# leotimus/binary-recommendation

Measured on NVIDIA B200. Metric: train interactions/sec (BPR, d=64, ML-1M shape), higher is better.
Workload: dtype f32

## Files before the change

binary-recommendation_b200/csrc/bpr.cu:

```cuda
#include "neumf_common.cuh"
#include <cooperative_groups.h>
#include <stdlib.h>
#include <vector>

namespace {

constexpr int kThreads = 256;

__device__ __forceinline__ uint32_t peek_touched(const uint32_t* touched, int64_t row) {
  return touched ? __ldg(touched + (row >> 5)) : 0xffffffffu;
}
__device__ __forceinline__ void mark_touched(uint32_t* touched, int64_t row, uint32_t seen) {
  const uint32_t bit = 1u << (row & 31);
  if (!(seen & bit)) atomicOr(touched + (row >> 5), bit);
}

__device__ __forceinline__ void finish_loss(double part, double inv_batch, double* acc, unsigned int* ticket,
                                            float* loss_out) {
  __shared__ double red[32];
  const double tot = block_sum_double(part, red);
  if (threadIdx.x == 0) {
    atomicAdd(acc, tot);
    __threadfence();
    const unsigned int t = atomicAdd(ticket, 1u);
    if (t == gridDim.x - 1) {
      __threadfence();
      const double sum = atomicAdd(acc, 0.0);
      if (loss_out) loss_out[0] = float(sum * inv_batch);
      *acc = 0.0;
      *ticket = 0u;
      __threadfence();
    }
  }
// ... 169 lines not shown
}

struct BprStep {
  int64_t off;
  int64_t sample_index;
  int32_t count;
  int32_t _pad;
};
constexpr int kInlineSteps = 16;
struct BprCoopParams {
  brk_table user, item;
  const int32_t* u; const int32_t* p; const int32_t* n;
  const BprStep* steps;
  BprStep inline_steps[kInlineSteps];
  int32_t use_inline;
  int32_t n_steps;
  brk_adam_hyper h;
  int64_t* state;
  float* losses;
  double* loss_acc;
  int32_t* stage;
  int64_t stage_pitch;
  const int64_t* csr_indptr; const int32_t* csr_items;
  uint32_t seed, epoch, num_items;
  float* const* peer_w; float* const* peer_g; uint32_t* const* peer_flags;
  float* dp_m; float* dp_v; uint32_t* dp_sync;
  int64_t arena_n4;
  int32_t rank, world;
  float inv_global;
  unsigned long long* dbg;
  long long spin_budget;
  int32_t prefetch;
  unsigned int* bar;
};

__device__ __forceinline__ void coop_st_release_sys(uint32_t* p, uint32_t v) {
  asm volatile("st.release.sys.global.u32 [%0], %1;" ::"l"(p), "r"(v) : "memory");
}
__device__ __forceinline__ bool coop_spin_sys(const uint32_t* p, uint32_t epoch, uint32_t* err, long long budget) {
  const long long t0 = clock64();
  while (true) {
    uint32_t v;
    asm volatile("ld.acquire.sys.global.u32 %0, [%1];" : "=r"(v) : "l"(p) : "memory");
    if (int32_t(v - epoch) >= 0) return true;
    if (clock64() - t0 > budget) { atomicExch(err, 1u); return false; }
    __nanosleep(32);
  }
}

__device__ __forceinline__ void coop_stamp(const BprCoopParams& P, int s, int k) {
  if (P.dbg && blockIdx.x == 0 && threadIdx.x == 0) {
    unsigned long long t;
    asm volatile("mov.u64 %0, %globaltimer;" : "=l"(t));
    P.dbg[s * 8 + k] = t;
  }
}

__device__ __forceinline__ void adam4(float4& w, float4& m, float4& v, const float4 g, float alpha, float b1, float b2,
                                      float eps) {
  const float omb1 = 1.f - b1, omb2 = 1.f - b2;
  m.x = b1 * m.x + omb1 * g.x; v.x = b2 * v.x + omb2 * g.x * g.x; w.x -= alpha * m.x / (sqrtf(v.x) + eps);
  m.y = b1 * m.y + omb1 * g.y; v.y = b2 * v.y + omb2 * g.y * g.y; w.y -= alpha * m.y / (sqrtf(v.y) + eps);
  m.z = b1 * m.z + omb1 * g.z; v.z = b2 * v.z + omb2 * g.z * g.z; w.z -= alpha * m.z / (sqrtf(v.z) + eps);
  m.w = b1 * m.w + omb1 * g.w; v.w = b2 * v.w + omb2 * g.w * g.w; w.w -= alpha * m.w / (sqrtf(v.w) + eps);
}

__device__ __forceinline__ void bpr_stage_step(const BprCoopParams& P, const BprStep sd, int slot, int64_t tid, int64_t nthr) {
  int32_t* su = P.stage + int64_t(slot) * 3 * P.stage_pitch;
  int32_t* sp = su + P.stage_pitch; int32_t* sn = sp + P.stage_pitch;
  for (int64_t b = tid; b < sd.count; b += nthr) {
    const int32_t uu = P.u[sd.off + b];
    su[b] = uu; sp[b] = P.p[sd.off + b];
    sn[b] = brk_sample_bpr_negative(uint64_t(sd.sample_index + b), uu, P.seed, P.epoch, P.num_items, P.csr_indptr, P.csr_items);
  }
}

constexpr int kStageThreads = 64;

template <int LPR, int NCH>
__global__ void __launch_bounds__(kThreads, 4) bpr_steps_coop(const BprCoopParams P) {
  namespace cg = cooperative_groups;
  cg::grid_group grid = cg::this_grid();
  unsigned int bar_target = P.bar ? *reinterpret_cast<volatile unsigned int*>(P.bar + 2) : 0u;
  auto gsync = [&]() {
    if (P.bar == nullptr) { grid.sync(); return; }
    __syncthreads();
    bar_target += gridDim.x;
    if (threadIdx.x == 0) {
      asm volatile("red.release.gpu.global.add.u32 [%0], 1;" ::"l"(P.bar) : "memory");
      const long long t0 = clock64();
      unsigned int v;
      do {
        asm volatile("ld.acquire.gpu.global.u32 %0, [%1];" : "=r"(v) : "l"(P.bar) : "memory");
        if (clock64() - t0 > 8000000000LL) { atomicExch(P.bar + 1, 1u); __trap(); }
      } while (int(v - bar_target) < 0);
    }
    __syncthreads();
  };
  auto gcollect = [&]() {
    if (P.bar == nullptr) { grid.sync(); return; }
    __syncthreads();
    bar_target += gridDim.x;
    if (threadIdx.x == 0) {
      asm volatile("red.release.gpu.global.add.u32 [%0], 1;" ::"l"(P.bar) : "memory");
      if (blockIdx.x == 0) {
        const long long t0 = clock64();
        unsigned int v;
        do {
          asm volatile("ld.acquire.gpu.global.u32 %0, [%1];" : "=r"(v) : "l"(P.bar) : "memory");
          if (clock64() - t0 > 8000000000LL) { atomicExch(P.bar + 1, 1u); __trap(); }
        } while (int(v - bar_target) < 0);
      }
    }
    if (blockIdx.x == 0) __syncthreads();
  };
  __shared__ double red[32];
  const bool sample = P.n == nullptr;
  const int d4 = P.user.d >> 2;
  const int lane_in = threadIdx.x & (LPR - 1);
  const int sub = (threadIdx.x & 31) / LPR;
  const int64_t group = (int64_t(blockIdx.x) * kThreads + threadIdx.x) / LPR;
  const int64_t n_groups = int64_t(gridDim.x) * kThreads / LPR;
  const int64_t warp_first = group - sub;
  const int64_t tid = int64_t(blockIdx.x) * kThreads + threadIdx.x, nthr = int64_t(gridDim.x) * kThreads;
  const float4* Wu4 = reinterpret_cast<const float4*>(P.user.w);
  const float4* Wi4 = reinterpret_cast<const float4*>(P.item.w);
  const double* pw = reinterpret_cast<const double*>(P.state);
  double p1 = pw[1], p2 = pw[2];
  const brk_table tabs[2] = {P.user, P.item};

  if (P.prefetch && threadIdx.x == 0) {
    for (int k = 0; k < 2; ++k) {
      const int64_t bytes = tabs[k].rows * tabs[k].d * 4;
      int64_t per = (bytes + gridDim.x - 1) / gridDim.x;
      per = (per + 15) & ~int64_t(15);
      const int64_t off = int64_t(blockIdx.x) * per;
      if (off < bytes) {
        const uint32_t n = uint32_t(((off + per <= bytes ? per : bytes - off)) & ~int64_t(15));
        if (n) {
          const float* arrs[4] = {tabs[k].w, tabs[k].g, P.world > 1 ? nullptr : tabs[k].m, P.world > 1 ? nullptr : tabs[k].v};
#pragma unroll
          for (int a = 0; a < 4; ++a)
            if (arrs[a] != nullptr && brk_aligned16(arrs[a]))
              asm volatile("cp.async.bulk.prefetch.L2.global [%0], %1;" ::"l"(reinterpret_cast<const char*>(arrs[a]) + off), "r"(n) : "memory");
        }
      }
    }
  }
  if (sample) {
    bpr_stage_step(P, P.use_inline ? P.inline_steps[0] : P.steps[0], 0, tid, nthr);
    gsync();
  }
  for (int s = 0; s < P.n_steps; ++s) {
    const BprStep sd = P.use_inline ? P.inline_steps[s] : P.steps[s];
    const int64_t batch = sd.count;
    const float inv_batch = P.world > 1 ? P.inv_global : 1.0f / float(batch);
    coop_stamp(P, s, 0);
    const int32_t *uid, *pid, *nid;
    if (sample) { uid = P.stage + int64_t(s & 1) * 3 * P.stage_pitch; pid = uid + P.stage_pitch; nid = pid + P.stage_pitch; }
    else { uid = P.u + sd.off; pid = P.p + sd.off; nid = P.n + sd.off; }
    float loss_local = 0.f;
    for (int64_t wb = warp_first; wb < batch; wb += n_groups) {
      const int64_t b = wb + sub;
      const bool valid = b < batch;
      int64_t ru = 0, rp = 0, rn = 0;
      if (valid) { ru = __ldcg(uid + b); rp = __ldcg(pid + b); rn = __ldcg(nid + b); }
      float4 u[NCH], p[NCH], n[NCH];
#pragma unroll
      for (int k = 0; k < NCH; ++k) {
        const int c = lane_in + k * LPR;
        if (valid && c < d4) {
          u[k] = __ldcg(Wu4 + ru * d4 + c); p[k] = __ldcg(Wi4 + rp * d4 + c); n[k] = __ldcg(Wi4 + rn * d4 + c);
        } else {
          u[k] = p[k] = n[k] = make_float4(0.f, 0.f, 0.f, 0.f);
        }
      }
      float dot = 0.f;
#pragma unroll
      for (int k = 0; k < NCH; ++k) {
        dot = fmaf(u[k].x, p[k].x - n[k].x, dot); dot = fmaf(u[k].y, p[k].y - n[k].y, dot);
        dot = fmaf(u[k].z, p[k].z - n[k].z, dot); dot = fmaf(u[k].w, p[k].w - n[k].w, dot);
      }
      const float x = group_sum<LPR>(dot);
      const float sg = sigmoidf_acc(x);
      if (valid && lane_in == 0) loss_local += 1.0f - sg;
      const float g = -sg * (1.0f - sg) * inv_batch;
      if (valid) {
#pragma unroll
        for (int k = 0; k < NCH; ++k) {
          const int c = lane_in + k * LPR;
          if (c < d4) {
            const float4 dp = make_float4(g * u[k].x, g * u[k].y, g * u[k].z, g * u[k].w);
            red_add_f4(P.user.g + (ru * d4 + c) * 4, make_float4(g * (p[k].x - n[k].x), g * (p[k].y - n[k].y),
                                                                 g * (p[k].z - n[k].z), g * (p[k].w - n[k].w)));
            red_add_f4(P.item.g + (rp * d4 + c) * 4, dp);
            red_add_f4(P.item.g + (rn * d4 + c) * 4, make_float4(-dp.x, -dp.y, -dp.z, -dp.w));
          }
        }
      }
    }
    const double part = block_sum_double(double(loss_local), red);
    if (threadIdx.x == 0) atomicAdd(P.loss_acc + (s & 1), part);
    if (P.world > 1) gcollect(); else gsync();
    coop_stamp(P, s, 1);
    p1 *= double(P.h.beta1); p2 *= double(P.h.beta2);
    const float alpha = float(double(P.h.lr) * sqrt(1.0 - p2) / (1.0 - p1));
    const bool staging = sample && s + 1 < P.n_steps;
    const bool stager = staging && threadIdx.x < kStageThreads;
    const int64_t atid = staging ? int64_t(blockIdx.x) * (kThreads - kStageThreads) + (threadIdx.x - kStageThreads) : tid;
    const int64_t anthr = staging ? int64_t(gridDim.x) * (kThreads - kStageThreads) : nthr;
    if (stager) {
      bpr_stage_step(P, P.use_inline ? P.inline_steps[s + 1] : P.steps[s + 1], (s + 1) & 1,
                     int64_t(blockIdx.x) * kStageThreads + threadIdx.x, int64_t(gridDim.x) * kStageThreads);
    }
    if (P.world == 1) {
      if (!stager) {
#pragma unroll
        for (int k = 0; k < 2; ++k) {
          const int64_t n4 = tabs[k].rows * tabs[k].d / 4;
          float4* w4 = reinterpret_cast<float4*>(tabs[k].w); float4* g4 = reinterpret_cast<float4*>(tabs[k].g);
          float4* m4 = reinterpret_cast<float4*>(tabs[k].m); float4* v4 = reinterpret_cast<float4*>(tabs[k].v);
          for (int64_t i = atid; i < n4; i += anthr) {
            float4 w = w4[i], m = m4[i], v = v4[i];
            adam4(w, m, v, g4[i], alpha, P.h.beta1, P.h.beta2, P.h.eps);
            w4[i] = w; m4[i] = m; v4[i] = v; g4[i] = make_float4(0.f, 0.f, 0.f, 0.f);
          }
        }
      }
    } else {
      const int G = P.world, me = P.rank;
      const uint32_t ep = P.dp_sync[3] + uint32_t(s) + 1u;
      uint32_t* my_flags = P.peer_flags[me];
      if (blockIdx.x == 0 && threadIdx.x < G) {
        __threadfence_system();
        coop_st_release_sys(P.peer_flags[threadIdx.x] + me, ep);
      }
      bool okA = true;
      if (threadIdx.x < G) okA = coop_spin_sys(my_flags + threadIdx.x, ep, P.dp_sync + 4, P.spin_budget);
      const bool deadA = __syncthreads_or(okA ? 0 : 1) != 0 || *reinterpret_cast<volatile uint32_t*>(P.dp_sync + 4) != 0u;
      coop_stamp(P, s, 2);
      if (!stager && !deadA) {
        const int64_t lo = P.arena_n4 * me / G, hi = P.arena_n4 * (me + 1) / G;
        float4* w_me = reinterpret_cast<float4*>(P.peer_w[me]);
        float4* m4 = reinterpret_cast<float4*>(P.dp_m); float4* v4 = reinterpret_cast<float4*>(P.dp_v);
        for (int64_t i = lo + atid; i < hi; i += anthr) {
          float4 g = make_float4(0.f, 0.f, 0.f, 0.f);
          for (int p = 0; p < G; ++p) {
            const float4 x = __ldcg(reinterpret_cast<const float4*>(P.peer_g[p]) + i);
            g.x += x.x; g.y += x.y; g.z += x.z; g.w += x.w;
          }
          float4 w = __ldcg(w_me + i), m = m4[i - lo], v = v4[i - lo];
          adam4(w, m, v, g, alpha, P.h.beta1, P.h.beta2, P.h.eps);
          m4[i - lo] = m; v4[i - lo] = v;
          w_me[i] = w;
        }
      }
      coop_stamp(P, s, 3);
      __threadfence();
      gcollect();
      coop_stamp(P, s, 4);
      const bool deadG = *reinterpret_cast<volatile uint32_t*>(P.dp_sync + 4) != 0u;
      if (!deadG && blockIdx.x == 0 && threadIdx.x < G) {
        __threadfence_system();
        coop_st_release_sys(P.peer_flags[threadIdx.x] + G + me, ep);
      }
      bool okB = true;
      if (!deadG && threadIdx.x < G) okB = coop_spin_sys(my_flags + G + threadIdx.x, ep, P.dp_sync + 4, P.spin_budget);
      const bool deadB = __syncthreads_or(okB ? 0 : 1) != 0 || deadG;
      coop_stamp(P, s, 5);
      if (!deadB) {
        float4* w_loc = reinterpret_cast<float4*>(P.peer_w[me]);
        const int64_t lo = P.arena_n4 * me / G, hi = P.arena_n4 * (me + 1) / G;
        const int64_t others = P.arena_n4 - (hi - lo);
        float4* g_me = reinterpret_cast<float4*>(P.peer_g[me]);
        for (int64_t i = tid; i < P.arena_n4; i += nthr) g_me[i] = make_float4(0.f, 0.f, 0.f, 0.f);
        for (int64_t j = tid; j < others; j += nthr) {
          const int64_t i = j < lo ? j : j + (hi - lo);
          int owner = int((i * G) / P.arena_n4);
          while (P.arena_n4 * owner / G > i) --owner;
          while (P.arena_n4 * (owner + 1) / G <= i) ++owner;
          w_loc[i] = __ldcg(reinterpret_cast<const float4*>(P.peer_w[owner]) + i);
        }
      }
    }
    if (tid == nthr - 1) {
      if (P.losses) P.losses[s] = float(P.loss_acc[s & 1] / double(batch));
      P.loss_acc[s & 1] = 0.0;
    }
    gsync();
    coop_stamp(P, s, 6);
    if (P.world > 1 && *reinterpret_cast<volatile uint32_t*>(P.dp_sync + 4) != 0u) break;
  }
  if (tid == 0 && !(P.world > 1 && *reinterpret_cast<volatile uint32_t*>(P.dp_sync + 4) != 0u)) {
    double* pwo = reinterpret_cast<double*>(P.state);
    P.state[0] += P.n_steps; pwo[1] = p1; pwo[2] = p2;
    if (P.world > 1) P.dp_sync[3] += uint32_t(P.n_steps);
    if (P.bar) P.bar[2] = bar_target;
  }
}

template <bool TRAIN>
int launch_bpr(brk_ctx* ctx, const float* Wu, const float* Wi, float* Gu, float* Gi, uint32_t* Tu, uint32_t* Ti,
               int d, const int32_t* u, const int32_t* p, const int32_t* n, int64_t batch, int64_t global_batch,
               float* out, cudaStream_t st) {
  const float inv_batch = 1.0f / float(global_batch > 0 ? global_batch : batch);
  const double inv_local = 1.0 / double(batch);
  double* acc = ctx->loss_acc + 0;
  unsigned int* ticket = ctx->tickets + 0;
  const int64_t cap = int64_t(ctx->sm_count) * (2048 / kThreads);
  const bool vec = (d & 3) == 0 && d <= 512 && brk_aligned16(Wu) && brk_aligned16(Wi) &&
                   (!TRAIN || (brk_aligned16(Gu) && brk_aligned16(Gi)));
  if (vec) {
    const int d4 = d >> 2;
    const int lpr = brk_lanes_per_row(d4);
    const int nch = (d4 + lpr - 1) / lpr;
    int64_t need = (batch * lpr + kThreads - 1) / kThreads;
    const int grid = int(need < 1 ? 1 : (need < cap ? need : cap));
#define BRK_BPR_CASE(L, N)                                                                          \
  bpr_vec<L, N, TRAIN><<<grid, kThreads, 0, st>>>(Wu, Wi, Gu, Gi, Tu, Ti, d4, u, p, n, batch, inv_batch, \
                                                  inv_local, acc, ticket, out)
    if (lpr == 1) BRK_BPR_CASE(1, 1);
    else if (lpr == 2) BRK_BPR_CASE(2, 1);
    else if (lpr == 4) BRK_BPR_CASE(4, 1);
    else if (lpr == 8) BRK_BPR_CASE(8, 1);
    else if (lpr == 16) BRK_BPR_CASE(16, 1);
    else if (nch == 1) BRK_BPR_CASE(32, 1);
    else if (nch == 2) BRK_BPR_CASE(32, 2);
    else if (nch == 3) BRK_BPR_CASE(32, 3);
// ... 87 lines not shown
    P.seed = P.epoch = P.num_items = 0;
  }
  if (dp && dp->world > 1) {
    P.peer_w = dp->peer_w; P.peer_g = dp->peer_g; P.peer_flags = dp->peer_flags; P.dp_m = dp->m; P.dp_v = dp->v;
    P.dp_sync = dp->local_sync; P.arena_n4 = dp->n / 4; P.rank = dp->rank; P.world = dp->world;
    P.inv_global = 1.0f / float(int64_t(dp->world) * max_count);
  } else {
    P.peer_w = nullptr; P.peer_g = nullptr; P.peer_flags = nullptr; P.dp_m = nullptr; P.dp_v = nullptr; P.dp_sync = nullptr;
    P.arena_n4 = 0; P.rank = 0; P.world = 1; P.inv_global = 0.f;
  }
  if (getenv("BRK_COOP_TRACE") && !g_coop_trace) {
    BRK_CUDA(cudaMalloc(&g_coop_trace, 4096 * 8 * sizeof(unsigned long long)));
    BRK_CUDA(cudaMemset(g_coop_trace, 0, 4096 * 8 * sizeof(unsigned long long)));
  }
  P.dbg = (g_coop_trace && n_steps <= 4096) ? g_coop_trace : nullptr;
  P.prefetch = getenv("BRK_BPR_NO_PREFETCH") ? 0 : 1;
  P.bar = getenv("BRK_BPR_CG_SYNC") ? nullptr : ctx->bpr_bar;
  {
    const char* e = getenv("BRK_PEER_SPIN_MS");
    const long long ms = e ? atoll(e) : 0;
    P.spin_budget = ms > 0 ? ms * 2000000LL : 60000000000LL;
  }
  const int lpr = brk_lanes_per_row(d >> 2);
  void* fn = nullptr;
  int slot = 0;
  switch (lpr) {
    case 1: fn = (void*)bpr_steps_coop<1, 1>; slot = 0; break;
    case 2: fn = (void*)bpr_steps_coop<2, 1>; slot = 1; break;
    case 4: fn = (void*)bpr_steps_coop<4, 1>; slot = 2; break;
    case 8: fn = (void*)bpr_steps_coop<8, 1>; slot = 3; break;
    case 16: fn = (void*)bpr_steps_coop<16, 1>; slot = 4; break;
    default: fn = (void*)bpr_steps_coop<32, 1>; slot = 5; break;
  }
  static int per_sm_cache[6] = {0, 0, 0, 0, 0, 0};
  int per_sm = per_sm_cache[slot];
  if (per_sm == 0) {
    BRK_CUDA(cudaOccupancyMaxActiveBlocksPerMultiprocessor(&per_sm, fn, kThreads, 0));
    BRK_REQUIRE(per_sm > 0, BRK_E_STATE, "brk_bpr_train_steps: cooperative kernel does not fit");
    per_sm_cache[slot] = per_sm;
  }
  int64_t want = (max_count * lpr + kThreads - 1) / kThreads;
  const int64_t cap = int64_t(per_sm) * ctx->sm_count;
  const int grid = int(want < cap ? (want < 1 ? 1 : want) : cap);
  void* args[] = {(void*)&P};
  BRK_CUDA(cudaLaunchCooperativeKernel(fn, dim3(grid), dim3(kThreads), args, 0, st));
  return 0;
}

static void make_steps(BprStep* out, const int64_t* batch_index, int n_steps, int64_t total, int64_t batch) {
  for (int k = 0; k < n_steps; ++k) {
    const int64_t off = batch_index[k] * batch;
    out[k].off = off; out[k].sample_index = off;
    out[k].count = int32_t((off + batch <= total) ? batch : total - off);
    out[k]._pad = 0;
  }
}

extern "C" int brk_bpr_train_steps(brk_ctx* ctx, const brk_table* user, const brk_table* item,
                                   const int32_t* u, const int32_t* p, const int32_t* n, int64_t total,
                                   int64_t batch, const int64_t* batch_index_host, int32_t n_steps,
                                   brk_adam_hyper h, int32_t lazy_adam, int64_t* step_dev, float* losses,
                                   void* stream) {
  BRK_REQUIRE(ctx && user && item && u && p && n && batch_index_host && step_dev, BRK_E_ARG,
              "brk_bpr_train_steps: null argument");
  BRK_REQUIRE(total > 0 && batch > 0 && n_steps >= 0, BRK_E_ARG, "brk_bpr_train_steps: total=%lld batch=%lld",
              (long long)total, (long long)batch);
  const int64_t n_batches = (total + batch - 1) / batch;
  for (int k = 0; k < n_steps; ++k)
    BRK_REQUIRE(batch_index_host[k] >= 0 && batch_index_host[k] < n_batches, BRK_E_ARG,
                "brk_bpr_train_steps: batch index %lld of %lld", (long long)batch_index_host[k], (long long)n_batches);
  if (n_steps == 0) return 0;
  cudaStream_t st = (cudaStream_t)stream;
  const bool coop_ok = coop_eligible(user, item, lazy_adam);
  if (coop_ok) {
    std::vector<BprStep> steps(n_steps);
    make_steps(steps.data(), batch_index_host, n_steps, total, batch);
    return launch_coop_steps(ctx, user, item, u, p, n, steps.data(), n_steps, batch < total ? batch : total, h, step_dev,
                             losses, st);
// ... 244 lines not shown
```

binary-recommendation_b200/csrc/tc.cuh:

```cuda
#pragma once
#include <cuda.h>
#include <cuda_runtime.h>
#include <stdint.h>

namespace tc {

__device__ __forceinline__ uint32_t smem_u32(const void* p) {
  return static_cast<uint32_t>(__cvta_generic_to_shared(p));
}

__device__ __forceinline__ void mbar_init(uint32_t bar, uint32_t count) {
  asm volatile("mbarrier.init.shared::cta.b64 [%0], %1;" ::"r"(bar), "r"(count));
}
__device__ __forceinline__ void fence_barrier_init() {
  asm volatile("fence.mbarrier_init.release.cluster;" ::: "memory");
}
__device__ __forceinline__ void mbar_expect_tx(uint32_t bar, uint32_t bytes) {
  asm volatile("mbarrier.arrive.expect_tx.shared::cta.b64 _, [%0], %1;" ::"r"(bar), "r"(bytes) : "memory");
}
__device__ __forceinline__ void mbar_arrive(uint32_t bar) {
  asm volatile("mbarrier.arrive.shared::cta.b64 _, [%0];" ::"r"(bar) : "memory");
}
__device__ __forceinline__ void mbar_wait(uint32_t bar, uint32_t parity) {
  asm volatile(
      "{\n"
      ".reg .pred p;\n"
      "MBAR_WAIT:\n"
      "mbarrier.try_wait.parity.shared::cta.b64 p, [%0], %1;\n"
      "@p bra MBAR_DONE;\n"
      "bra MBAR_WAIT;\n"
      "MBAR_DONE:\n"
      "}\n" ::"r"(bar), "r"(parity) : "memory");
}

__device__ __forceinline__ void prefetch_tensormap(const CUtensorMap* m) {
  asm volatile("prefetch.tensormap [%0];" ::"l"(reinterpret_cast<uint64_t>(m)) : "memory");
}
__device__ __forceinline__ void tma_load_2d(uint32_t smem_dst, const CUtensorMap* m, int c0, int c1, uint32_t bar) {
  asm volatile(
      "cp.async.bulk.tensor.2d.shared::cluster.global.mbarrier::complete_tx::bytes [%0], [%1, {%3, %4}], [%2];"
      ::"r"(smem_dst), "l"(reinterpret_cast<uint64_t>(m)), "r"(bar), "r"(c0), "r"(c1) : "memory");
}

template <int COLS>
__device__ __forceinline__ void tmem_alloc(uint32_t smem_slot) {
  asm volatile("tcgen05.alloc.cta_group::1.sync.aligned.shared::cta.b32 [%0], %1;" ::"r"(smem_slot), "n"(COLS) : "memory");
  asm volatile("tcgen05.relinquish_alloc_permit.cta_group::1.sync.aligned;" ::: "memory");
}
template <int COLS>
__device__ __forceinline__ void tmem_dealloc(uint32_t taddr) {
  asm volatile("tcgen05.dealloc.cta_group::1.sync.aligned.b32 %0, %1;" ::"r"(taddr), "n"(COLS) : "memory");
}
__device__ __forceinline__ void fence_before_sync() { asm volatile("tcgen05.fence::before_thread_sync;" ::: "memory"); }
__device__ __forceinline__ void fence_after_sync() { asm volatile("tcgen05.fence::after_thread_sync;" ::: "memory"); }

__device__ __forceinline__ uint64_t smem_desc_sw128(uint32_t smem_addr) {
  uint64_t d = 0;
  d |= uint64_t((smem_addr >> 4) & 0x3FFFu);
  d |= uint64_t(1) << 16;
  d |= uint64_t(1024 >> 4) << 32;
  d |= uint64_t(1) << 46;
  d |= uint64_t(2) << 61;
  return d;
}
__device__ __forceinline__ uint64_t smem_desc_sw128_ex(uint32_t smem_addr, uint32_t lbo_bytes, uint32_t sbo_bytes) {
  uint64_t d = 0;
  d |= uint64_t((smem_addr >> 4) & 0x3FFFu);
  d |= uint64_t((lbo_bytes >> 4) & 0x3FFFu) << 16;
  d |= uint64_t((sbo_bytes >> 4) & 0x3FFFu) << 32;
  d |= uint64_t(1) << 46;
  d |= uint64_t(2) << 61;
  return d;
}
__device__ __forceinline__ uint64_t smem_desc_sw128_base32(uint32_t smem_addr, uint32_t lbo_bytes, uint32_t sbo_bytes) {
// ... 119 lines not shown
```

Baseline: 725.2 million.

## Keep embedding and Adam moment slabs resident in shared memory across coop steps

When both tables fit in a 48 KB per-block budget, each block of the cooperative BPR kernel bulk-loads its slice of weights and Adam m/v into shared memory at entry, using an mbarrier. The Adam update then runs from shared memory with gradients staged through cp.async, and m/v are written back only on the last step. This is meant to cut repeated global traffic for the optimizer state. It also narrows index math to 32-bit, keeps the bias-correction powers in shared memory, skips the trailing grid barrier on the last single-GPU step, and adds a tracing script. In exchange it forces the grid to full residency and adds shared-memory pressure and setup latency.

Result: faster. 764.2 million, median of 6 (+5.4%).

```diff
diff --git a/binary-recommendation_b200/csrc/bpr.cu b/binary-recommendation_b200/csrc/bpr.cu
--- a/binary-recommendation_b200/csrc/bpr.cu
+++ b/binary-recommendation_b200/csrc/bpr.cu
@@ -1,4 +1,5 @@
 #include "neumf_common.cuh"
+#include "tc.cuh"
 #include <cooperative_groups.h>
 #include <stdlib.h>
 #include <vector>
@@ -234,6 +235,7 @@
   long long spin_budget;
   int32_t prefetch;
   unsigned int* bar;
+  int32_t slab_pitch;
 };
 
 __device__ __forceinline__ void coop_st_release_sys(uint32_t* p, uint32_t v) {
@@ -278,11 +280,13 @@
 }
 
 constexpr int kStageThreads = 64;
+constexpr size_t kSlabBudget = 48 << 10;
 
 template <int LPR, int NCH>
 __global__ void __launch_bounds__(kThreads, 4) bpr_steps_coop(const BprCoopParams P) {
   namespace cg = cooperative_groups;
   cg::grid_group grid = cg::this_grid();
+  coop_stamp(P, 0, 7);
   unsigned int bar_target = P.bar ? *reinterpret_cast<volatile unsigned int*>(P.bar + 2) : 0u;
   auto gsync = [&]() {
     if (P.bar == nullptr) { grid.sync(); return; }
@@ -321,15 +325,47 @@
   const int d4 = P.user.d >> 2;
   const int lane_in = threadIdx.x & (LPR - 1);
   const int sub = (threadIdx.x & 31) / LPR;
-  const int64_t group = (int64_t(blockIdx.x) * kThreads + threadIdx.x) / LPR;
-  const int64_t n_groups = int64_t(gridDim.x) * kThreads / LPR;
-  const int64_t warp_first = group - sub;
-  const int64_t tid = int64_t(blockIdx.x) * kThreads + threadIdx.x, nthr = int64_t(gridDim.x) * kThreads;
+  const int n_groups = int(gridDim.x) * (kThreads / LPR);
+  const int warp_first = int(blockIdx.x) * (kThreads / LPR) + int(threadIdx.x) / LPR - sub;
+  const int tid = int(blockIdx.x) * kThreads + int(threadIdx.x), nthr = int(gridDim.x) * kThreads;
   const float4* Wu4 = reinterpret_cast<const float4*>(P.user.w);
   const float4* Wi4 = reinterpret_cast<const float4*>(P.item.w);
   const double* pw = reinterpret_cast<const double*>(P.state);
-  double p1 = pw[1], p2 = pw[2];
+  __shared__ __align__(16) double bpow[2][2];
+  if (threadIdx.x == 0) {
+    asm volatile("cp.async.ca.shared.global [%0], [%1], 8;" ::"r"(tc::smem_u32(&bpow[0][0])), "l"(pw + 1) : "memory");
+    asm volatile("cp.async.ca.shared.global [%0], [%1], 8;" ::"r"(tc::smem_u32(&bpow[0][1])), "l"(pw + 2) : "memory");
+  }
   const brk_table tabs[2] = {P.user, P.item};
+
+  extern __shared__ __align__(16) float4 slab[];
+  __shared__ __align__(8) uint64_t slab_bar;
+  __shared__ int64_t slab_lo[2];
+  __shared__ int slab_cnt[2];
+  const bool onchip = P.slab_pitch > 0;
+  if (onchip && threadIdx.x == 0) {
+    const uint32_t bar = tc::smem_u32(&slab_bar);
+    int64_t lo[2]; int c[2];
+#pragma unroll
+    for (int k = 0; k < 2; ++k) {
+      const uint32_t n4 = uint32_t(tabs[k].rows * d4);
+      lo[k] = n4 * blockIdx.x / gridDim.x;
+      c[k] = int(n4 * (blockIdx.x + 1) / gridDim.x - uint32_t(lo[k]));
+      slab_lo[k] = lo[k]; slab_cnt[k] = c[k];
+    }
+    tc::mbar_init(bar, 1);
+    tc::fence_proxy_async_smem();
+    tc::mbar_expect_tx(bar, uint32_t(c[0] + c[1]) * 3u * 16u);
+#pragma unroll
+    for (int k = 0; k < 2; ++k) {
+      if (c[k] == 0) continue;
+      const float* arrs[3] = {tabs[k].w, tabs[k].m, tabs[k].v};
+#pragma unroll
+      for (int a = 0; a < 3; ++a)
+        tc::bulk_load(tc::smem_u32(slab + a * P.slab_pitch + (k == 0 ? 0 : c[0])),
+                      reinterpret_cast<const float4*>(arrs[a]) + lo[k], uint32_t(c[k]) * 16u, bar);
+    }
+  }
 
   if (P.prefetch && threadIdx.x == 0) {
     for (int k = 0; k < 2; ++k) {
@@ -340,7 +376,8 @@
       if (off < bytes) {
         const uint32_t n = uint32_t(((off + per <= bytes ? per : bytes - off)) & ~int64_t(15));
         if (n) {
-          const float* arrs[4] = {tabs[k].w, tabs[k].g, P.world > 1 ? nullptr : tabs[k].m, P.world > 1 ? nullptr : tabs[k].v};
+          const bool mv = P.world == 1 && !onchip;
+          const float* arrs[4] = {onchip ? nullptr : tabs[k].w, tabs[k].g, mv ? tabs[k].m : nullptr, mv ? tabs[k].v : nullptr};
 #pragma unroll
           for (int a = 0; a < 4; ++a)
             if (arrs[a] != nullptr && brk_aligned16(arrs[a]))
@@ -355,15 +392,15 @@
   }
   for (int s = 0; s < P.n_steps; ++s) {
     const BprStep sd = P.use_inline ? P.inline_steps[s] : P.steps[s];
-    const int64_t batch = sd.count;
+    const int batch = sd.count;
     const float inv_batch = P.world > 1 ? P.inv_global : 1.0f / float(batch);
     coop_stamp(P, s, 0);
     const int32_t *uid, *pid, *nid;
     if (sample) { uid = P.stage + int64_t(s & 1) * 3 * P.stage_pitch; pid = uid + P.stage_pitch; nid = pid + P.stage_pitch; }
     else { uid = P.u + sd.off; pid = P.p + sd.off; nid = P.n + sd.off; }
     float loss_local = 0.f;
-    for (int64_t wb = warp_first; wb < batch; wb += n_groups) {
-      const int64_t b = wb + sub;
+    for (int wb = warp_first; wb < batch; wb += n_groups) {
+      const int b = wb + sub;
       const bool valid = b < batch;
       int64_t ru = 0, rp = 0, rn = 0;
       if (valid) { ru = __ldcg(uid + b); rp = __ldcg(pid + b); rn = __ldcg(nid + b); }
@@ -402,10 +439,14 @@
       }
     }
     const double part = block_sum_double(double(loss_local), red);
-    if (threadIdx.x == 0) atomicAdd(P.loss_acc + (s & 1), part);
+    if (threadIdx.x == 0) {
+      atomicAdd(P.loss_acc + (s & 1), part);
+      asm volatile("cp.async.wait_all;" ::: "memory");
+    }
     if (P.world > 1) gcollect(); else gsync();
     coop_stamp(P, s, 1);
-    p1 *= double(P.h.beta1); p2 *= double(P.h.beta2);
+    const double p1 = bpow[s & 1][0] * double(P.h.beta1), p2 = bpow[s & 1][1] * double(P.h.beta2);
+    if (threadIdx.x == 0) { bpow[(s + 1) & 1][0] = p1; bpow[(s + 1) & 1][1] = p2; }
     const float alpha = float(double(P.h.lr) * sqrt(1.0 - p2) / (1.0 - p1));
     const bool staging = sample && s + 1 < P.n_steps;
     const bool stager = staging && threadIdx.x < kStageThreads;
@@ -415,7 +456,35 @@
       bpr_stage_step(P, P.use_inline ? P.inline_steps[s + 1] : P.steps[s + 1], (s + 1) & 1,
                      int64_t(blockIdx.x) * kStageThreads + threadIdx.x, int64_t(gridDim.x) * kStageThreads);
     }
-    if (P.world == 1) {
+    const bool last = s + 1 == P.n_steps;
+    if (onchip) {
+      if (!stager) {
+        tc::mbar_wait(tc::smem_u32(&slab_bar), 0);
+        const int la = staging ? threadIdx.x - kStageThreads : threadIdx.x;
+        const int nla = staging ? kThreads - kStageThreads : kThreads;
+        const int64_t lo0 = slab_lo[0], lo1 = slab_lo[1];
+        const int cnt0 = slab_cnt[0], cnt = cnt0 + slab_cnt[1];
+        float4* gs = slab + 3 * P.slab_pitch;
+        for (int j = la; j < cnt; j += nla) {
+          const bool it = j >= cnt0;
+          const float4* src = reinterpret_cast<const float4*>(it ? P.item.g : P.user.g) + (it ? lo1 + (j - cnt0) : lo0 + j);
+          asm volatile("cp.async.cg.shared.global [%0], [%1], 16;" ::"r"(tc::smem_u32(gs + j)), "l"(src) : "memory");
+        }
+        asm volatile("cp.async.wait_all;" ::: "memory");
+        for (int j = la; j < cnt; j += nla) {
+          const bool it = j >= cnt0;
+          const brk_table& T = it ? P.item : P.user;
+          const int64_t i = it ? lo1 + (j - cnt0) : lo0 + j;
+          float4 w = slab[j], m = slab[P.slab_pitch + j], v = slab[2 * P.slab_pitch + j];
+          adam4(w, m, v, gs[j], alpha, P.h.beta1, P.h.beta2, P.h.eps);
+          slab[j] = w; slab[P.slab_pitch + j] = m; slab[2 * P.slab_pitch + j] = v;
+          reinterpret_cast<float4*>(T.w)[i] = w;
+          reinterpret_cast<float4*>(T.g)[i] = make_float4(0.f, 0.f, 0.f, 0.f);
+          if (last) { reinterpret_cast<float4*>(T.m)[i] = m; reinterpret_cast<float4*>(T.v)[i] = v; }
+        }
+      }
+      coop_stamp(P, s, 2);
+    } else if (P.world == 1) {
       if (!stager) {
 #pragma unroll
         for (int k = 0; k < 2; ++k) {
@@ -429,6 +498,7 @@
           }
         }
       }
+      coop_stamp(P, s, 2);
     } else {
       const int G = P.world, me = P.rank;
       const uint32_t ep = P.dp_sync[3] + uint32_t(s) + 1u;
@@ -489,13 +559,13 @@
       if (P.losses) P.losses[s] = float(P.loss_acc[s & 1] / double(batch));
       P.loss_acc[s & 1] = 0.0;
     }
-    gsync();
+    if (!(last && P.world == 1)) gsync();
     coop_stamp(P, s, 6);
     if (P.world > 1 && *reinterpret_cast<volatile uint32_t*>(P.dp_sync + 4) != 0u) break;
   }
   if (tid == 0 && !(P.world > 1 && *reinterpret_cast<volatile uint32_t*>(P.dp_sync + 4) != 0u)) {
     double* pwo = reinterpret_cast<double*>(P.state);
-    P.state[0] += P.n_steps; pwo[1] = p1; pwo[2] = p2;
+    P.state[0] += P.n_steps; pwo[1] = bpow[P.n_steps & 1][0]; pwo[2] = bpow[P.n_steps & 1][1];
     if (P.world > 1) P.dp_sync[3] += uint32_t(P.n_steps);
     if (P.bar) P.bar[2] = bar_target;
   }
@@ -649,18 +719,48 @@
     case 16: fn = (void*)bpr_steps_coop<16, 1>; slot = 4; break;
     default: fn = (void*)bpr_steps_coop<32, 1>; slot = 5; break;
   }
-  static int per_sm_cache[6] = {0, 0, 0, 0, 0, 0};
-  int per_sm = per_sm_cache[slot];
-  if (per_sm == 0) {
-    BRK_CUDA(cudaOccupancyMaxActiveBlocksPerMultiprocessor(&per_sm, fn, kThreads, 0));
-    BRK_REQUIRE(per_sm > 0, BRK_E_STATE, "brk_bpr_train_steps: cooperative kernel does not fit");
-    per_sm_cache[slot] = per_sm;
-  }
-  int64_t want = (max_count * lpr + kThreads - 1) / kThreads;
-  const int64_t cap = int64_t(per_sm) * ctx->sm_count;
-  const int grid = int(want < cap ? (want < 1 ? 1 : want) : cap);
+  static int per_sm_cache[2][6] = {{0, 0, 0, 0, 0, 0}, {0, 0, 0, 0, 0, 0}};
+  auto resident = [&](int with_slab, int* out) -> int {
+    int per_sm = per_sm_cache[with_slab][slot];
+    if (per_sm == 0) {
+      const size_t smem = with_slab ? kSlabBudget : 0;
+      if (with_slab) BRK_CUDA(cudaFuncSetAttribute(fn, cudaFuncAttributeMaxDynamicSharedMemorySize, int(kSlabBudget)));
+      BRK_CUDA(cudaOccupancyMaxActiveBlocksPerMultiprocessor(&per_sm, fn, kThreads, smem));
+      BRK_REQUIRE(per_sm > 0, BRK_E_STATE, "brk_bpr_train_steps: cooperative kernel does not fit (%zu B shared)", smem);
+      per_sm_cache[with_slab][slot] = per_sm;
+    }
+    *out = per_sm;
+    return 0;
+  };
+  int grid = 0;
+  size_t smem = 0;
+  P.slab_pitch = 0;
+  const brk_table* tb[2] = {user, item};
+  bool slab_ok = P.world == 1;
+  for (int k = 0; k < 2; ++k) slab_ok = slab_ok && brk_aligned16(tb[k]->m) && brk_aligned16(tb[k]->v);
+  if (slab_ok) {
+    int per_sm = 0;
+    if (int rc = resident(1, &per_sm)) return rc;
+    const int64_t g = int64_t(per_sm) * ctx->sm_count;
+    int64_t pitch4 = 0;
+    bool fits32 = true;
+    for (int k = 0; k < 2; ++k) {
+      pitch4 += (tb[k]->rows * (d >> 2) + g - 1) / g;
+      fits32 = fits32 && tb[k]->rows * (d >> 2) * g < (int64_t(1) << 32);
+    }
+    if (fits32 && pitch4 * 4 * 16 <= int64_t(kSlabBudget)) {
+      grid = int(g); P.slab_pitch = int32_t(pitch4); smem = size_t(pitch4) * 4 * 16;
+    }
+  }
+  if (grid == 0) {
+    int per_sm = 0;
+    if (int rc = resident(0, &per_sm)) return rc;
+    int64_t want = (max_count * lpr + kThreads - 1) / kThreads;
+    const int64_t cap = int64_t(per_sm) * ctx->sm_count;
+    grid = int(want < cap ? (want < 1 ? 1 : want) : cap);
+  }
   void* args[] = {(void*)&P};
-  BRK_CUDA(cudaLaunchCooperativeKernel(fn, dim3(grid), dim3(kThreads), args, 0, st));
+  BRK_CUDA(cudaLaunchCooperativeKernel(fn, dim3(grid), dim3(kThreads), args, smem, st));
   return 0;
 }
 
diff --git a/binary-recommendation_b200/csrc/tc.cuh b/binary-recommendation_b200/csrc/tc.cuh
--- a/binary-recommendation_b200/csrc/tc.cuh
+++ b/binary-recommendation_b200/csrc/tc.cuh
@@ -40,6 +40,10 @@
   asm volatile(
       "cp.async.bulk.tensor.2d.shared::cluster.global.mbarrier::complete_tx::bytes [%0], [%1, {%3, %4}], [%2];"
       ::"r"(smem_dst), "l"(reinterpret_cast<uint64_t>(m)), "r"(bar), "r"(c0), "r"(c1) : "memory");
+}
+__device__ __forceinline__ void bulk_load(uint32_t smem_dst, const void* src, uint32_t bytes, uint32_t bar) {
+  asm volatile("cp.async.bulk.shared::cluster.global.mbarrier::complete_tx::bytes [%0], [%1], %2, [%3];"
+               ::"r"(smem_dst), "l"(src), "r"(bytes), "r"(bar) : "memory");
 }
 
 template <int COLS>
diff --git a/profiles/bpr_trace.py b/profiles/bpr_trace.py
--- /dev/null
+++ b/profiles/bpr_trace.py
@@ -0,0 +1,84 @@
+import os, sys, ctypes, subprocess
+KERNEL_TIME = "--kernel-time" in sys.argv
+if not KERNEL_TIME:
+    os.environ["BRK_COOP_TRACE"] = "1"
+ROOT = os.path.dirname(os.path.dirname(os.path.abspath(__file__))); sys.path.insert(0, ROOT)
+import numpy as np, torch
+from binrec_b200 import synth
+from binrec_b200 import _native as N
+from binrec_b200.BPRModel import BPRNet
+
+dev = torch.device("cuda:0")
+users, items = synth.make_interactions()
+net = BPRNet(synth.ML1M_USERS, synth.ML1M_ITEMS, 64, seed=42, learning_rate=1e-3, sparse_adam="keras", device=dev)
+net.set_training_pairs(users, items); net.sample_negatives(7, 0)
+B = 16384
+n_batches = len(users) // B
+flush = torch.empty((256 << 20) // 4, dtype=torch.float32, device=dev)
+sink = torch.empty(1024, dtype=torch.float32, device=dev); ssum = torch.empty((), dtype=torch.float32, device=dev)
+lib = N.lib(); lib.brk_coop_trace_read.argtypes = [ctypes.c_void_p, ctypes.c_int32]
+
+
+def flush_l2():
+    flush.zero_(); sink.copy_(flush[:sink.numel()] + flush[-sink.numel():]); torch.sum(flush, dim=0, out=ssum)
+
+
+def read(k):
+    buf = (ctypes.c_uint64 * (k * 8))()
+    assert lib.brk_coop_trace_read(buf, k * 8) == 0
+    return np.frombuffer(buf, dtype=np.uint64).reshape(k, 8).astype(np.int64)
+
+
+def span(a, i, j):
+    return (a[..., j] - a[..., i]) / 1e3
+
+
+if KERNEL_TIME:
+    from torch.profiler import profile, ProfilerActivity
+    for k in range(5):
+        flush_l2(); net.train_steps([k % n_batches], B)
+    torch.cuda.synchronize()
+    K = 50
+    with profile(activities=[ProfilerActivity.CUDA]) as prof:
+        for k in range(K):
+            flush_l2(); net.train_steps([(5 + k) % n_batches], B)
+        torch.cuda.synchronize()
+    ts = [e.time_range.elapsed_us() for e in prof.events()
+          if e.device_type == torch.autograd.DeviceType.CUDA and "bpr_steps_coop" in e.name]
+    print(f"\n[torch.profiler, separate run, no stamps] bpr_steps_coop, {len(ts)} flushed single-step launches: "
+          f"mean {np.mean(ts):.2f} us  median {np.median(ts):.2f}  min {np.min(ts):.2f}")
+    sys.exit(0)
+
+print(f"{torch.cuda.get_device_name(0)}; block-0 %globaltimer stamps, mean / median in us")
+for k in range(5):
+    flush_l2(); net.train_steps([k % n_batches], B)
+torch.cuda.synchronize()
+K = 50
+rows = []
+for k in range(K):
+    flush_l2(); net.train_steps([(5 + k) % n_batches], B); torch.cuda.synchronize()
+    rows.append(read(1)[0])
+a = np.array(rows)
+phases = [("entry -> step start (slot 7 -> 0)", 7, 0), ("phase 1 + first barrier (0 -> 1)", 0, 1),
+          ("Adam, thread 0 of block 0 (1 -> 2)", 1, 2), ("rest of the step (2 -> 6)", 2, 6),
+          ("Adam + trailing barrier (1 -> 6)", 1, 6), ("whole launch, block 0 (7 -> 6)", 7, 6)]
+print(f"\n[flushed] {K} single-step launches, L2 flushed before each")
+for name, i, j in phases:
+    x = span(a, i, j)
+    print(f"  {name:40s} mean {x.mean():6.2f}  median {np.median(x):6.2f}  min {x.min():6.2f}")
+
+S = 40
+order = [k % n_batches for k in range(S)]
+net.train_steps(order, B); torch.cuda.synchronize()
+net.train_steps(order, B); torch.cuda.synchronize()
+h = read(S)
+print(f"\n[hot] one {S}-step launch, back to back")
+print(f"  {'entry -> step 0 start (7 -> 0)':40s} {span(h[0], 7, 0):6.2f}")
+for name, i, j in phases[1:5]:
+    x = span(h, i, j)
+    print(f"  {name:40s} step 0 {x[0]:6.2f}  steps 1..{S - 1} mean {x[1:].mean():6.2f}  last {x[-1]:6.2f}")
+print(f"  {'step to step (0 -> next 0)':40s} mean {((h[1:, 0] - h[:-1, 0]) / 1e3).mean():6.2f}")
+print(f"  {'whole launch, block 0 (7 -> last 6)':40s} {(h[-1, 6] - h[0, 7]) / 1e3:6.2f}  = {(h[-1, 6] - h[0, 7]) / 1e3 / S:.2f} per step")
+
+sys.stdout.flush()
+subprocess.run([sys.executable, os.path.abspath(__file__), "--kernel-time"], check=True)
```

## Keep dense Adam m/v/w slices resident in shared memory across coop steps

Applied to the files above, without the earlier changes.

When each block's slice of the user and item tables fits in shared memory, the cooperative BPR kernel bulk-loads its w/m/v slice once with TMA (cp.async.bulk plus an mbarrier). It then runs the per-step dense Adam update from shared memory and writes m and v back only at kernel exit. This removes the repeated global reads of w, m and v and the global writes of m and v on every step. It also skips the final grid barrier, moves the beta powers into shared memory and narrows the index arithmetic to 32-bit. In exchange the kernel needs large dynamic shared memory, which may limit occupancy, and correctness now depends on the slice math and the single-GPU path. A profiling script for per-phase tracing is added.

Result: faster. 729.4 million before, 783.5 million after, median of 6 (+7.4%).

```diff
diff --git a/binary-recommendation_b200/csrc/bpr.cu b/binary-recommendation_b200/csrc/bpr.cu
--- a/binary-recommendation_b200/csrc/bpr.cu
+++ b/binary-recommendation_b200/csrc/bpr.cu
@@ -234,6 +234,8 @@
   long long spin_budget;
   int32_t prefetch;
   unsigned int* bar;
+  int32_t slice4[2];
+  int32_t last_sync;
 };
 
 __device__ __forceinline__ void coop_st_release_sys(uint32_t* p, uint32_t v) {
@@ -278,6 +280,13 @@
 }
 
 constexpr int kStageThreads = 64;
+
+__device__ __forceinline__ bool coop_mbar_try_wait(uint32_t bar, uint32_t parity) {
+  uint32_t ok;
+  asm volatile("{\n.reg .pred p;\nmbarrier.try_wait.parity.shared::cta.b64 p, [%1], %2;\nselp.u32 %0, 1, 0, p;\n}\n"
+               : "=r"(ok) : "r"(bar), "r"(parity) : "memory");
+  return ok != 0;
+}
 
 template <int LPR, int NCH>
 __global__ void __launch_bounds__(kThreads, 4) bpr_steps_coop(const BprCoopParams P) {
@@ -321,30 +330,53 @@
   const int d4 = P.user.d >> 2;
   const int lane_in = threadIdx.x & (LPR - 1);
   const int sub = (threadIdx.x & 31) / LPR;
-  const int64_t group = (int64_t(blockIdx.x) * kThreads + threadIdx.x) / LPR;
-  const int64_t n_groups = int64_t(gridDim.x) * kThreads / LPR;
-  const int64_t warp_first = group - sub;
-  const int64_t tid = int64_t(blockIdx.x) * kThreads + threadIdx.x, nthr = int64_t(gridDim.x) * kThreads;
+  const int group = int(blockIdx.x * kThreads + threadIdx.x) / LPR;
+  const int n_groups = int(gridDim.x) * kThreads / LPR;
+  const int warp_first = group - sub;
+  const int tid = int(blockIdx.x * kThreads + threadIdx.x), nthr = int(gridDim.x) * kThreads;
   const float4* Wu4 = reinterpret_cast<const float4*>(P.user.w);
   const float4* Wi4 = reinterpret_cast<const float4*>(P.item.w);
   const double* pw = reinterpret_cast<const double*>(P.state);
-  double p1 = pw[1], p2 = pw[2];
+  __shared__ double beta_pow[2][2];
+  if (threadIdx.x == 0) { beta_pow[0][0] = pw[1]; beta_pow[0][1] = pw[2]; }
   const brk_table tabs[2] = {P.user, P.item};
 
-  if (P.prefetch && threadIdx.x == 0) {
+  extern __shared__ float4 adam_smem[];
+  __shared__ __align__(8) uint64_t adam_bar;
+  const bool smem_adam = P.slice4[0] > 0;
+  coop_stamp(P, 0, 7);
+  if (P.dbg && P.world == 1 && blockIdx.x == 0 && threadIdx.x == 0) P.dbg[4] = smem_adam ? 1u : 0u;
+  if (threadIdx.x == 0) {
+    const uint32_t bar = uint32_t(__cvta_generic_to_shared(&adam_bar));
+    if (smem_adam) {
+      asm volatile("mbarrier.init.shared::cta.b64 [%0], 1;" ::"r"(bar) : "memory");
+      asm volatile("fence.mbarrier_init.release.cluster;\n\tfence.proxy.async.shared::cta;" ::: "memory");
+    }
+    uint32_t nb[2], tx = 0;
+    int64_t offs[2];
+#pragma unroll
     for (int k = 0; k < 2; ++k) {
       const int64_t bytes = tabs[k].rows * tabs[k].d * 4;
-      int64_t per = (bytes + gridDim.x - 1) / gridDim.x;
+      int64_t per = smem_adam ? int64_t(P.slice4[k]) * 16 : (bytes + gridDim.x - 1) / gridDim.x;
       per = (per + 15) & ~int64_t(15);
-      const int64_t off = int64_t(blockIdx.x) * per;
-      if (off < bytes) {
-        const uint32_t n = uint32_t(((off + per <= bytes ? per : bytes - off)) & ~int64_t(15));
-        if (n) {
-          const float* arrs[4] = {tabs[k].w, tabs[k].g, P.world > 1 ? nullptr : tabs[k].m, P.world > 1 ? nullptr : tabs[k].v};
-#pragma unroll
-          for (int a = 0; a < 4; ++a)
-            if (arrs[a] != nullptr && brk_aligned16(arrs[a]))
-              asm volatile("cp.async.bulk.prefetch.L2.global [%0], %1;" ::"l"(reinterpret_cast<const char*>(arrs[a]) + off), "r"(n) : "memory");
+      offs[k] = int64_t(blockIdx.x) * per;
+      nb[k] = offs[k] < bytes ? uint32_t((offs[k] + per <= bytes ? per : bytes - offs[k]) & ~int64_t(15)) : 0u;
+      tx += nb[k];
+    }
+    if (smem_adam) asm volatile("mbarrier.arrive.expect_tx.shared::cta.b64 _, [%0], %1;" ::"r"(bar), "r"(3 * tx) : "memory");
+#pragma unroll
+    for (int k = 0; k < 2; ++k) {
+      if (nb[k] == 0) continue;
+      const float* arrs[4] = {tabs[k].g, tabs[k].w, P.world > 1 ? nullptr : tabs[k].m, P.world > 1 ? nullptr : tabs[k].v};
+#pragma unroll
+      for (int a = 0; a < 4; ++a) {
+        const char* src = reinterpret_cast<const char*>(arrs[a]) + offs[k];
+        if (smem_adam && a > 0) {
+          const uint32_t dst = uint32_t(__cvta_generic_to_shared(adam_smem)) + (a - 1) * tx + (k ? nb[0] : 0u);
+          asm volatile("cp.async.bulk.shared::cluster.global.mbarrier::complete_tx::bytes [%0], [%1], %2, [%3];"
+                       ::"r"(dst), "l"(src), "r"(nb[k]), "r"(bar) : "memory");
+        } else if (P.prefetch && arrs[a] != nullptr && brk_aligned16(arrs[a])) {
+          asm volatile("cp.async.bulk.prefetch.L2.global [%0], %1;" ::"l"(src), "r"(nb[k]) : "memory");
         }
       }
     }
@@ -362,8 +394,8 @@
     if (sample) { uid = P.stage + int64_t(s & 1) * 3 * P.stage_pitch; pid = uid + P.stage_pitch; nid = pid + P.stage_pitch; }
     else { uid = P.u + sd.off; pid = P.p + sd.off; nid = P.n + sd.off; }
     float loss_local = 0.f;
-    for (int64_t wb = warp_first; wb < batch; wb += n_groups) {
-      const int64_t b = wb + sub;
+    for (int wb = warp_first; wb < batch; wb += n_groups) {
+      const int b = wb + sub;
       const bool valid = b < batch;
       int64_t ru = 0, rp = 0, rn = 0;
       if (valid) { ru = __ldcg(uid + b); rp = __ldcg(pid + b); rn = __ldcg(nid + b); }
@@ -403,19 +435,53 @@
     }
     const double part = block_sum_double(double(loss_local), red);
     if (threadIdx.x == 0) atomicAdd(P.loss_acc + (s & 1), part);
-    if (P.world > 1) gcollect(); else gsync();
+    if (P.world > 1) {
+      gcollect();
+    } else {
+      coop_stamp(P, s, 2);
+      gsync();
+    }
     coop_stamp(P, s, 1);
-    p1 *= double(P.h.beta1); p2 *= double(P.h.beta2);
+    const double p1 = beta_pow[s & 1][0] * double(P.h.beta1), p2 = beta_pow[s & 1][1] * double(P.h.beta2);
+    if (threadIdx.x == 0) { beta_pow[(s + 1) & 1][0] = p1; beta_pow[(s + 1) & 1][1] = p2; }
     const float alpha = float(double(P.h.lr) * sqrt(1.0 - p2) / (1.0 - p1));
     const bool staging = sample && s + 1 < P.n_steps;
     const bool stager = staging && threadIdx.x < kStageThreads;
-    const int64_t atid = staging ? int64_t(blockIdx.x) * (kThreads - kStageThreads) + (threadIdx.x - kStageThreads) : tid;
-    const int64_t anthr = staging ? int64_t(gridDim.x) * (kThreads - kStageThreads) : nthr;
+    const int atid = staging ? int(blockIdx.x) * (kThreads - kStageThreads) + (int(threadIdx.x) - kStageThreads) : tid;
+    const int anthr = staging ? int(gridDim.x) * (kThreads - kStageThreads) : nthr;
     if (stager) {
       bpr_stage_step(P, P.use_inline ? P.inline_steps[s + 1] : P.steps[s + 1], (s + 1) & 1,
                      int64_t(blockIdx.x) * kStageThreads + threadIdx.x, int64_t(gridDim.x) * kStageThreads);
     }
-    if (P.world == 1) {
+    if (P.world == 1 && smem_adam) {
+      if (s == 0) {
+        const uint32_t bar = uint32_t(__cvta_generic_to_shared(&adam_bar));
+        while (!coop_mbar_try_wait(bar, 0)) {}
+      }
+      if (!stager) {
+        int64_t o4[2];
+        int n4[2];
+#pragma unroll
+        for (int k = 0; k < 2; ++k) {
+          const int64_t tot = tabs[k].rows * tabs[k].d / 4;
+          o4[k] = int64_t(blockIdx.x) * P.slice4[k];
+          n4[k] = o4[k] < tot ? int(tot - o4[k] < P.slice4[k] ? tot - o4[k] : P.slice4[k]) : 0;
+        }
+        const int nA = n4[0] + n4[1];
+        float4* sw = adam_smem; float4* sm = sw + nA; float4* sv = sm + nA;
+        const int t0 = staging ? int(threadIdx.x) - kStageThreads : int(threadIdx.x);
+        const int T = staging ? kThreads - kStageThreads : kThreads;
+        for (int j = t0; j < nA; j += T) {
+          const bool u = j < n4[0];
+          float4* w4 = reinterpret_cast<float4*>(u ? P.user.w : P.item.w) + (u ? o4[0] + j : o4[1] + (j - n4[0]));
+          float4* g4 = reinterpret_cast<float4*>(u ? P.user.g : P.item.g) + (u ? o4[0] + j : o4[1] + (j - n4[0]));
+          float4 w = sw[j], m = sm[j], v = sv[j];
+          adam4(w, m, v, __ldcg(g4), alpha, P.h.beta1, P.h.beta2, P.h.eps);
+          sw[j] = w; sm[j] = m; sv[j] = v;
+          *w4 = w; *g4 = make_float4(0.f, 0.f, 0.f, 0.f);
+        }
+      }
+    } else if (P.world == 1) {
       if (!stager) {
 #pragma unroll
         for (int k = 0; k < 2; ++k) {
@@ -489,13 +555,39 @@
       if (P.losses) P.losses[s] = float(P.loss_acc[s & 1] / double(batch));
       P.loss_acc[s & 1] = 0.0;
     }
-    gsync();
+    if (P.world == 1) coop_stamp(P, s, 3);
+    if (P.world > 1 || s + 1 < P.n_steps || P.last_sync) gsync();
     coop_stamp(P, s, 6);
     if (P.world > 1 && *reinterpret_cast<volatile uint32_t*>(P.dp_sync + 4) != 0u) break;
   }
+  if (smem_adam) {
+    asm volatile("fence.proxy.async.shared::cta;" ::: "memory");
+    __syncthreads();
+    if (threadIdx.x == 0) {
+      uint32_t nb[2];
+#pragma unroll
+      for (int k = 0; k < 2; ++k) {
+        const int64_t bytes = tabs[k].rows * tabs[k].d * 4, off = int64_t(blockIdx.x) * P.slice4[k] * 16;
+        nb[k] = off < bytes ? uint32_t(bytes - off < int64_t(P.slice4[k]) * 16 ? bytes - off : int64_t(P.slice4[k]) * 16) : 0u;
+      }
+      const uint32_t base = uint32_t(__cvta_generic_to_shared(adam_smem)), tx = nb[0] + nb[1];
+#pragma unroll
+      for (int k = 0; k < 2; ++k) {
+        if (nb[k] == 0) continue;
+        const int64_t off = int64_t(blockIdx.x) * P.slice4[k] * 16;
+        float* dsts[2] = {tabs[k].m, tabs[k].v};
+#pragma unroll
+        for (int a = 0; a < 2; ++a)
+          asm volatile("cp.async.bulk.global.shared::cta.bulk_group [%0], [%1], %2;"
+                       ::"l"(reinterpret_cast<char*>(dsts[a]) + off), "r"(base + (a + 1) * tx + (k ? nb[0] : 0u)), "r"(nb[k])
+                       : "memory");
+      }
+      asm volatile("cp.async.bulk.commit_group;\n\tcp.async.bulk.wait_group 0;" ::: "memory");
+    }
+  }
   if (tid == 0 && !(P.world > 1 && *reinterpret_cast<volatile uint32_t*>(P.dp_sync + 4) != 0u)) {
     double* pwo = reinterpret_cast<double*>(P.state);
-    P.state[0] += P.n_steps; pwo[1] = p1; pwo[2] = p2;
+    P.state[0] += P.n_steps; pwo[1] = beta_pow[P.n_steps & 1][0]; pwo[2] = beta_pow[P.n_steps & 1][1];
     if (P.world > 1) P.dp_sync[3] += uint32_t(P.n_steps);
     if (P.bar) P.bar[2] = bar_target;
   }
@@ -650,17 +742,35 @@
     default: fn = (void*)bpr_steps_coop<32, 1>; slot = 5; break;
   }
   static int per_sm_cache[6] = {0, 0, 0, 0, 0, 0};
+  static size_t smem_cap_cache[6] = {0, 0, 0, 0, 0, 0};
   int per_sm = per_sm_cache[slot];
   if (per_sm == 0) {
     BRK_CUDA(cudaOccupancyMaxActiveBlocksPerMultiprocessor(&per_sm, fn, kThreads, 0));
     BRK_REQUIRE(per_sm > 0, BRK_E_STATE, "brk_bpr_train_steps: cooperative kernel does not fit");
+    size_t cap_bytes = 0;
+    BRK_CUDA(cudaOccupancyAvailableDynamicSMemPerBlock(&cap_bytes, fn, per_sm, kThreads));
     per_sm_cache[slot] = per_sm;
+    smem_cap_cache[slot] = cap_bytes;
   }
   int64_t want = (max_count * lpr + kThreads - 1) / kThreads;
   const int64_t cap = int64_t(per_sm) * ctx->sm_count;
   const int grid = int(want < cap ? (want < 1 ? 1 : want) : cap);
+  size_t smem = 0;
+  const brk_table* tabs[2] = {user, item};
+  for (int k = 0; k < 2; ++k) {
+    const int64_t n4 = tabs[k]->rows * d / 4;
+    const int64_t s4 = (n4 + grid - 1) / grid;
+    P.slice4[k] = int32_t(s4 < (int64_t(1) << 20) ? s4 : 0);
+    smem += 3 * size_t(s4) * 16;
+  }
+  const bool smem_ok = P.world == 1 && !getenv("BRK_BPR_NO_SMEM_ADAM") && smem <= smem_cap_cache[slot] &&
+                       P.slice4[0] > 0 && P.slice4[1] > 0 && brk_aligned16(user->m) && brk_aligned16(user->v) &&
+                       brk_aligned16(item->m) && brk_aligned16(item->v);
+  if (!smem_ok) { P.slice4[0] = P.slice4[1] = 0; smem = 0; }
+  P.last_sync = getenv("BRK_BPR_NO_SMEM_ADAM") ? 1 : 0;
+  if (smem > 48 * 1024) BRK_CUDA(cudaFuncSetAttribute(fn, cudaFuncAttributeMaxDynamicSharedMemorySize, int(smem)));
   void* args[] = {(void*)&P};
-  BRK_CUDA(cudaLaunchCooperativeKernel(fn, dim3(grid), dim3(kThreads), args, 0, st));
+  BRK_CUDA(cudaLaunchCooperativeKernel(fn, dim3(grid), dim3(kThreads), args, smem, st));
   return 0;
 }
 
diff --git a/profiles/bpr_phase_trace.py b/profiles/bpr_phase_trace.py
--- /dev/null
+++ b/profiles/bpr_phase_trace.py
@@ -0,0 +1,96 @@
+import argparse, ctypes, json, os, subprocess, sys
+ROOT = os.path.dirname(os.path.dirname(os.path.abspath(__file__))); sys.path.insert(0, ROOT)
+os.environ["BRK_COOP_TRACE"] = "1"
+import numpy as np, torch
+from binrec_b200 import synth, _native as N
+from binrec_b200.BPRModel import BPRNet
+
+B, D, HOT_STEPS = 16384, 64, 40
+MODES = {"global": "1", "smem": None}
+
+
+def set_mode(m):
+    if MODES[m]: os.environ["BRK_BPR_NO_SMEM_ADAM"] = MODES[m]
+    else: os.environ.pop("BRK_BPR_NO_SMEM_ADAM", None)
+
+
+def read_trace(n_steps):
+    buf = (ctypes.c_uint64 * (n_steps * 8))()
+    assert N.lib().brk_coop_trace_read(buf, n_steps * 8) == 0
+    return np.frombuffer(buf, dtype=np.uint64).reshape(n_steps, 8).astype(np.int64)
+
+
+def phases(a):
+    return {"phase1": (a[:, 2] - a[:, 0]) / 1e3, "barrier_a": (a[:, 1] - a[:, 2]) / 1e3,
+            "adam": (a[:, 3] - a[:, 1]) / 1e3, "barrier_b": (a[:, 6] - a[:, 3]) / 1e3}
+
+
+def med(d):
+    return {k: round(float(np.median(v)), 3) for k, v in d.items()}
+
+
+def main():
+    ap = argparse.ArgumentParser()
+    ap.add_argument("--launches", type=int, default=200)
+    ap.add_argument("--json", default=None)
+    args = ap.parse_args()
+    dev = torch.device("cuda:0")
+    lib = N.lib(); lib.brk_coop_trace_read.argtypes = [ctypes.c_void_p, ctypes.c_int32]
+    try:
+        gpu = subprocess.run(["nvidia-smi", "--query-gpu=name,power.limit", "--format=csv,noheader", "-i", "0"],
+                             capture_output=True, text=True, timeout=30).stdout.strip()
+    except Exception:
+        gpu = torch.cuda.get_device_name(0)
+    users, items = synth.make_interactions()
+    net = BPRNet(synth.ML1M_USERS, synth.ML1M_ITEMS, D, seed=42, device=dev)
+    net.set_training_pairs(users, items); net.sample_negatives(7, 0)
+    nb = len(users) // B
+    flush = torch.empty((256 << 20) // 4, dtype=torch.float32, device=dev)
+    out = {"gpu": gpu, "shape": {"users": synth.ML1M_USERS, "items": synth.ML1M_ITEMS, "d": D, "batch": B}}
+
+    for m in MODES:
+        set_mode(m); net.train_steps(list(range(3)), B)
+    torch.cuda.synchronize()
+    rows = {m: [] for m in MODES}; ev_us = {m: [] for m in MODES}
+    e0, e1 = torch.cuda.Event(enable_timing=True), torch.cuda.Event(enable_timing=True)
+    for k in range(2 * args.launches):
+        m = list(MODES)[k % 2]
+        set_mode(m)
+        flush.zero_(); torch.sum(flush, dim=0)
+        e0.record(); net.train_steps([k % nb], B); e1.record()
+        torch.cuda.synchronize()
+        a = read_trace(1)
+        rows[m].append(a[0]); ev_us[m].append(1e3 * e0.elapsed_time(e1))
+    out["flushed"] = {}
+    for m in MODES:
+        a = np.stack(rows[m])
+        r = med(phases(a))
+        r["startup"] = round(float(np.median((a[:, 0] - a[:, 7]) / 1e3)), 3)
+        r["entry_to_end"] = round(float(np.median((a[:, 6] - a[:, 7]) / 1e3)), 3)
+        r["step_event"] = round(float(np.median(ev_us[m])), 3)
+        r["launches_on_smem_adam"] = int((a[:, 4] == 1).sum())
+        out["flushed"][m] = r
+
+    out["hot"] = {}
+    order = [k % nb for k in range(HOT_STEPS)]
+    samples = {m: [] for m in MODES}
+    for rep in range(10):
+        for m in MODES:
+            set_mode(m)
+            net.train_steps(order, B); torch.cuda.synchronize()
+            samples[m].append(read_trace(HOT_STEPS))
+    for m in MODES:
+        a = np.stack(samples[m][1:])
+        inner = a[:, :-1].reshape(-1, 8)
+        r = {"steps_but_last": med(phases(inner)), "last_step": med(phases(a[:, -1])),
+             "step_period": round(float(np.median(np.diff(a[:, :, 0], axis=1)) / 1e3), 3)}
+        out["hot"][m] = r
+    set_mode("smem")
+    print(json.dumps(out, indent=1))
+    if args.json:
+        with open(args.json, "w") as f:
+            json.dump(out, f, indent=1)
+
+
+if __name__ == "__main__":
+    main()
```
